# burchim/EfficientConformer

Measured on AMD Instinct MI355X. Metric: audio-frames/sec through encoder, EffConformerCTC-Small, 1/2/4/8 GPU, higher is better.
Workload: dtype bf16; 1 GPU; EfficientConformerCTCSmall: bf16 operands / fp32 accumulate, B=256 utterances/GPU (the largest single-GPU batch measured; SURVEY.md 8d lists B in {4, 32, 128}: --batch 128 is 0.79 x this rate, profiles/r5_31_bench_b128.json), lognormal 1.5-16 s (LibriSpeech-shaped), sorted desc; ragged: every utterance at its own length in one concatenated row space per row range (no pad frames; outputs = the refe; global_batch=256, streams_per_gpu=3, parallelism=dp1 (utterance shards), row_ranges=3 ragged row range(s) per GPU, cut for equal valid frames

## Files before the change

efficientconformer_amd/csrc/encoder.hip:

```cpp
#include "forward_common.h"
#include "pack.h"
#include "routes.h"

#include <cstring>

namespace {

thread_local std::string g_err;

}

int ec_fail(const char* msg) { g_err = msg ? msg : "error"; return -1; }

const void* ec_upload(EcEncoder* e, const void* src, size_t used) {
    if (e->dry) {
        static const char nowhere[16] = {0};
        const unsigned char* p = static_cast<const unsigned char*>(src);
        uint64_t h = 0xcbf29ce484222325ull ^ used;
        size_t i = 0;
        for (; i + 8 <= used; i += 8) { uint64_t w; memcpy(&w, p + i, 8); h = (h ^ w) * 0x100000001b3ull; h ^= h >> 29; }
        for (; i < used; ++i) h = (h ^ p[i]) * 0x100000001b3ull;
        e->dry->sum += h * 0x9E3779B97F4A7C15ull + 1; e->dry->buffers += 1; e->dry->bytes += (int64_t)used;
        return nowhere;
    }
// ... 12 lines not shown

int forward_dispatch(EcEncoder* e, const float* in, const int64_t* in_len, int from_audio, int n, const Shapes& s, float* out, int out_frames, int64_t* out_len,
                     void* workspace, size_t workspace_bytes, hipStream_t st) {
    char* ws = reinterpret_cast<char*>(workspace);
    const size_t mel_bytes = from_audio ? al((size_t)s.B * e->cfg.n_mels * s.Tm * 4) : 0;
    Workspace w; XWorkspace xw;
    size_t mel_off;
    if (e->exact_on) { xw = make_xworkspace(e, s); mel_off = xw.total; }
    else { w = make_workspace(e, s, from_audio != 0); mel_off = w.mel; }
    if (workspace_bytes < (e->exact_on ? xw.total + mel_bytes : w.total)) return fail("workspace too small");
    const float* mel = in;
    if (from_audio) {
        float* m = reinterpret_cast<float*>(ws + mel_off);
        PROF(PC_MEL, 0, (double)s.B * n * 4 + (double)s.B * e->cfg.n_mels * s.Tm * 4);
        EC_ABL(s.ragged && !e->exact_on ? 16 : 0, EC_TRY(launch_mel(in, s.B, n, e->mel, e->cfg.n_fft, e->cfg.hop_length, e->cfg.n_mels, s.Tm, e->cfg.normalize,
                                                                    e->cfg.mean, e->cfg.std, m, st, s.ragged ? in_len : nullptr)));
        mel = m;
    }
    if (e->exact_on) return forward_exact(e, mel, in_len, from_audio, s, xw, ws, out, out_len, st, out_frames);
    return forward_core(e, mel, in_len, from_audio, s, w, ws, out, out_len, st, out_frames);
}

bool ragged_host_lengths(const EcEncoder* e, const int64_t* host_len, int32_t batch, int32_t n, int32_t from_audio, std::vector<int>* tm) {
    tm->resize(batch);
    for (int b = 0; b < batch; ++b) {
        const int64_t l = host_len[b];
        if (l > n || (from_audio ? l <= e->cfg.n_fft / 2 : l < 1)) return false;
        (*tm)[b] = from_audio ? (int)(l / e->cfg.hop_length + 1) : (int)l;
    }
    return true;
}
// ... 110 lines not shown
    if (!x || !x_len || !x_len_host || !out || !workspace || batch <= 0 || n <= 0 || out_frames <= 0) return fail("bad argument");
    std::vector<int> tm;
    if (!ragged_host_lengths(e, x_len_host, batch, n, from_audio, &tm)) return fail("ragged lengths out of range (audio: n_fft / 2 < len <= n; mel: 1 <= len <= n)");
    Shapes s = make_shapes_ragged(e, tm);
    if (s.Tout.back() > out_frames) return fail("out_frames smaller than the longest utterance's output");
    s.Tm = from_audio ? n / e->cfg.hop_length + 1 : n;
    return forward_dispatch(e, x, x_len, from_audio, n, s, out, out_frames, out_len, workspace, workspace_bytes, (hipStream_t)stream);
}

int effconf_mel_frontend(EcEncoder* e, const float* audio, int32_t batch, int32_t n_samples, float* mel, void* stream) {
    if (!e || !e->finalized) return fail("encoder not finalized");
    if (!audio || !mel) return fail("mel_frontend: null argument");
    if (batch > 0 && n_samples <= e->cfg.n_fft / 2) return fail("mel_frontend: n_samples must exceed n_fft / 2 (reflect padding)");
    const int Tm = n_samples / e->cfg.hop_length + 1;
    EC_TRY(launch_mel(audio, batch, n_samples, e->mel, e->cfg.n_fft, e->cfg.hop_length, e->cfg.n_mels, Tm,
                      e->cfg.normalize, e->cfg.mean, e->cfg.std, mel, (hipStream_t)stream));
    return 0;
}

int effconf_ctc_greedy(EcEncoder* e, const float* enc_out, const int64_t* out_len, int32_t batch, int32_t t_out,
                       int32_t* labels, int32_t* label_len, float* logits, void* workspace, size_t workspace_bytes, void* stream) {
    if (!e || !e->finalized) return fail("encoder not finalized");
    if (!e->fc_wt) return fail("no CTC head (fc.weight / fc.bias) loaded");
    if (workspace_bytes < (size_t)batch * t_out * 4) return fail("workspace too small");
    int* preds = reinterpret_cast<int*>(workspace);
    hipStream_t st = (hipStream_t)stream;
    const int mode = e->exact_on && e->ctc_mfma == 2 ? 1 : e->ctc_mfma;
    if (mode == 2 && e->fc_hi && launch_ctc_split(enc_out, batch * t_out, e->blocks.back().dim_expand, e->fc_hi, e->fc_lo, e->fc_b, e->cfg.vocab_size,
                                                  preds, logits, st) == 0) {
    } else
    EC_TRY(launch_ctc_argmax(enc_out, batch * t_out, e->blocks.back().dim_expand, e->fc_wt, e->fc_b, e->cfg.vocab_size,
// ... 85 lines not shown
    e->ic_out.assign(probs, probs + n);
    return 0;
}

int effconf_encoder_set_option(EcEncoder* e, const char* name, int32_t value) {
    if (!e || !name) return fail("null argument");
    if (!strcmp(name, "fuse_subsample")) { if (value < 0 || value > 3) return fail("fuse_subsample: 0, 1, 2 or 3"); e->fuse_subsample = value; return 0; }
    if (!strcmp(name, "fuse_chain")) { e->fuse_chain = value != 0; return 0; }
    if (!strcmp(name, "ctc_mfma")) { if (value < 0 || value > 2) return fail("ctc_mfma: 0 (VALU), 1 (fp32 MFMA) or 2 (split-bf16 MFMA)"); e->ctc_mfma = value; return 0; }
    if (!strcmp(name, "wide_gemm")) { if (value < 0 || (value > 3 && value < 16)) return fail("wide_gemm: 0 (by shape), 1 (never), 2 (256-column tile), 3 (128-column tile), >= 16 (by shape with this many 256 x 256 tiles as the threshold)"); e->wide_gemm = value; return 0; }
    if (!strcmp(name, "attention_v2")) { if (value != 0 && value != 1 && value != 2) return fail("attention_v2: 0, 1 or 2"); e->attention_v2 = value; return 0; }
    if (!strcmp(name, "chain_full_max")) { if (value < 0 || value > 256) return fail("chain_full_max: widest stage (0..256) that runs chain A as ONE kernel"); e->chain_full_max = value; return 0; }
    if (!strcmp(name, "chain_max_dim")) { e->chain_max_dim = value; return 0; }
    if (!strcmp(name, "chain_small_m")) { e->chain_small_m = value; return 0; }
    if (!strcmp(name, "chain_pair")) { if (value != 0 && value != 5) return fail("chain_pair: 0 (chain.hip everywhere) or 5 (chain3.hip for chain A, chain2.hip for chain B at padded width 256)"); e->chain_pair = value; return 0; }
    if (!strcmp(name, "dwconv_mfma")) { if (value < 0 || value > 2) return fail("dwconv_mfma: 0, 1 (kernel size 15) or 2 (15 / 31 / 7)"); e->dwconv_mfma = value; return 0; }
    if (!strcmp(name, "tiled_min_k")) { e->tiled_min_k = value; return 0; }
    if (!strcmp(name, "tiled_auto")) { e->tiled_auto = value; return 0; }
    if (!strcmp(name, "split_ffn")) { e->split_ffn = value != 0; return 0; }
    if (!strcmp(name, "split_sublin")) { e->split_sublin = value != 0; return 0; }
    if (!strcmp(name, "sub3_auto")) { e->sub3_auto = value != 0; return 0; }
    if (!strcmp(name, "split_chain")) { e->split_chain = value != 0; return 0; }
    if (!strcmp(name, "trace_fused")) { e->trace_fused = value != 0; return 0; }
    if (!strcmp(name, "exact_attention")) { if (value < 0 || value > 2) return fail("exact_attention: 0 (tiled), 2 (tiled, 16-row workgroups) or 1 (one wave per query row)"); e->exact_attention = value; return 0; }
    if (!strcmp(name, "cache_pos_embeddings")) { e->e_cache_on = value != 0; e->e_cache.clear(); return 0; }
    if (!strcmp(name, "exact_fp32")) {
        if (!e->finalized) { e->exact_pack = e->exact_on = value != 0; e->exact_split = value == 2; return 0; }
        if (value && !e->exact_pack) return fail("exact_fp32 must be requested before effconf_encoder_finalize (the fp32 weights are uploaded there)");
        if (value == 2 && e->xsplit.empty()) return fail("exact_fp32 = 2 must be requested before effconf_encoder_finalize (the split weight images are built there)");
        e->exact_on = value != 0; e->exact_split = value == 2;
// ... 42 lines not shown
```

efficientconformer_amd/csrc/encoder_state.h:

```cpp
#pragma once
#include "kernels.h"
#include "../../include/effconf.h"

#include <map>
#include <string>
#include <vector>

int ec_fail(const char* msg);
inline int fail(const std::string& m) { return ec_fail(m.c_str()); }
#define EC_TRY(expr) do { int _rc = (expr); if (_rc != 0) return fail(std::string(#expr) + " failed rc=" + std::to_string(_rc)); } while (0)

inline int ld8(int d) { return ec_round_up(d, 8); }

struct HostTensor { std::vector<float> data; std::vector<int64_t> shape; };

struct PackedLinear { const bf16_t* w = nullptr; const float* bias = nullptr; int N = 0, K = 0, ldw = 0; std::vector<float> hbias;  };
struct SubChunkImg { const uint16_t *cimg = nullptr, *wimg = nullptr; const float* bias = nullptr; int ncb = 0, fo = 0; };
struct LNp { const float* g = nullptr; const float* b = nullptr; };

struct BlockW {
    LNp ln_ffn1, ln_att, ln_conv, ln_ffn2, ln_out;
    PackedLinear ffn1_a, ffn1_b, qkv, qkv_nat, pos, outp, pw1, pw2, res, ffn2_a, ffn2_b;
    const bf16_t *ffn1_bp = nullptr, *ffn2_bp = nullptr;
    const float *u = nullptr, *v = nullptr, *dw_w = nullptr, *dw_b = nullptr;
// ... 28 lines not shown
    PackDigest* dry = nullptr;
    size_t guard_bytes = 0;
    const float *sub_w9 = nullptr, *sub_b = nullptr;
    PackedLinear lin;
    const bf16_t* lin_fused = nullptr; int lin_fused_ld = 0;
    SubChunkImg sub3, xsub;
    const bf16_t* lin_rs = nullptr; const float* conv_tab = nullptr;
    int fuse_subsample = 2;
    bool fuse_chain = true;
    int ctc_mfma = 2;
    int attention_v2 = 1;
    int chain_full_max = 192;
    int dwconv_mfma = 1;
    int chain_pair = 5;
    int chain_small_m = 4096;
    int chain_max_dim = 256;
    int tiled_auto = 1;
    bool tiled_auto_on = false;
    int tiled_min_k = 256;
    std::vector<float*> att_out;
    int split_chain = 1;
    int sub3_auto = 1;
    int split_sublin = 1;
    int split_ffn = 1;
    bool trace_fused = false;
    int exact_attention = 0;
    const bf16_t* sub2_w = nullptr; const float* sub2_b = nullptr; int sub2_cp = 0;
    std::vector<BlockW> bw;
    const float *fc_wt = nullptr, *fc_b = nullptr;
    const bf16_t *fc_hi = nullptr, *fc_lo = nullptr;
// ... 51 lines not shown
```

efficientconformer_amd/csrc/forward_bf16.hip:

```cpp
#include "forward_common.h"
#include "routes.h"
#include "stream.h"

#include <cmath>

Workspace make_workspace(const EcEncoder* e, const Shapes& s, bool from_audio) {
    Workspace w;
    size_t off = 0;
    auto take = [&](size_t bytes) { size_t o = off; off += al(bytes); return o; };
    const size_t B = s.B;
    size_t mx = 0, ma = 0, mh = 0, mq = 0, me = 0, mg = 0, mc = 0;
    std::vector<size_t> esz;
    for (size_t k = 0; k < e->blocks.size(); ++k) {
        const EcBlock& b = e->blocks[k];
        const size_t T = s.Tin[k], D = b.dim_model, De = b.dim_expand;
        const size_t Tp = ec_round_up((int)T, b.group_size), Tg = Tp / b.group_size;
        const size_t d = (size_t)b.group_size * D / b.num_heads, dpad = ec_round_up((int)d, 32);
        const size_t Mi = (size_t)s.Min[k], Mo = (size_t)s.Mout[k], Mqk = (size_t)s.Mq[k];
        mx = std::max(mx, std::max(Mi * D, Mo * De) * 4);
        ma = std::max(ma, std::max(Mi * ld8(D), Mo * ld8(De)) * 2);
        mh = std::max(mh, std::max(Mi * D, Mo * De) * b.ff_ratio * 2);
        mq = std::max(mq, Mqk * D * 2 + 512);
        me = std::max(me, (size_t)b.num_heads * (2 * Tg - 1) * dpad * 2);
        esz.push_back((size_t)b.num_heads * (2 * Tg - 1) * dpad * 2 + 512);
// ... 92 lines not shown
    if (route == FRONT_TWO_LAYER) {
        const int T2 = (Tl1 - 1) / 2 + 1, F1 = c.n_mels / 2, F2q = c.n_mels / 4, C1 = c.sub_filters[1];
        { PROF(PC_SUBCONV, 2.0 * 9 * B * Tl1 * (double)C0 * F1, (double)B * c.n_mels * Tm * 4 + (double)B * Tl1 * F1 * e->sub2_cp * 2);
          EC_TRY(launch_subsample_conv_cl(mel, B, c.n_mels, Tm, Tl1, e->sub_w9, e->sub_b, C0, e->sub2_cp, act1, st, mel_len)); }
        trace_add(e, st, "subsample1", act1, (int64_t)B * F1 * Tl1, C0, e->sub2_cp, 1);
        { PROF(PC_GEMM_OTHER, 2.0 * 9 * (double)B * F2q * T2 * C0 * C1, (double)B * Tl1 * F1 * e->sub2_cp * 2 + (double)B * T2 * F2q * C1 * 2);
          EC_TRY(launch_conv2_igemm(act1, B, F1, Tl1, e->sub2_cp, e->sub2_w, 9 * e->sub2_cp, e->sub2_b, C1, F2q, T2, sub, st)); }
        trace_add(e, st, "subsample", sub, (int64_t)B * T2, F2q * C1, F2q * C1, 1);
        EC_TRY(run_gemm(e, PC_GEMM_OTHER, st, sub, F2q * C1, B * T2, e->lin, EPI_F32, rg ? xrect : x, N));
        if (rg) { PROF(PC_MISC, 0, Mr * N * 8); EC_TRY(launch_gather_rows(xrect, N, T2, r0, x, st)); }
    } else if (route == FRONT_CHUNKED) {
        PROF(PC_SUBCONV, 2.0 * 9 * Mr * Ksub + 2.0 * Mr * Ksub * N, (double)B * c.n_mels * Tm * 4 + Mr * N * 4);
        EC_TRY(launch_sublinear3(sub_chunk_params(e, e->sub3, mel, s, rg, x), st));
    } else if (route == FRONT_ROW_STAT) {
        PROF(PC_SUBCONV, 2.0 * 9 * Mr * Ksub + 2.0 * Mr * Ksub * N, (double)B * c.n_mels * Tm * 4 + Mr * N * 4);
        EC_ABL(rg ? 32 : 0, EC_TRY(launch_sublinear2(mel, B, c.n_mels, Tm, s.T1, e->conv_tab, e->lin_rs, e->lin.bias, C0, N, x, N, st, rg ? &r0 : nullptr, mel_len)));
    } else if (route == FRONT_TILED_FUSED) {
        PROF(PC_SUBCONV, 2.0 * 9 * Mr * Ksub + 2.0 * Mr * Ksub * N, (double)B * c.n_mels * Tm * 4 + Mr * N * 4);
        EC_TRY(launch_sublinear_fused(mel, B, c.n_mels, Tm, s.T1, e->sub_w9, e->sub_b, C0, e->lin_fused, e->lin_fused_ld, e->lin.bias, N, x, N, st));
    } else {
        const int Tcover = rg ? Tl1 + e->blocks[0].group_size - 1 : s.T1;
        { PROF(PC_SUBCONV, 2.0 * 9 * Mr * Ksub, (double)B * c.n_mels * Tm * 4 + Mr * Ksub * 2);
          EC_TRY(launch_subsample_conv(mel, B, c.n_mels, Tm, Tcover, e->sub_w9, e->sub_b, C0, sub, Ksub, st, mel_len, rg ? &r0 : nullptr)); }
        trace_add(e, st, "subsample", sub, s.Min[0], Ksub, Ksub, 1);
        EC_TRY(run_gemm(e, PC_GEMM_OTHER, st, sub, Ksub, (int)s.Min[0], e->lin, EPI_F32, x, N));
    }
    return 0;
}

ChainParams chain_params(const EcEncoder* e) { ChainParams cp{}; cp.small_m = e->chain_small_m; cp.pair = e->chain_pair; return cp; }

// ... 351 lines not shown
```

efficientconformer_amd/csrc/kernels.h:

```cpp
#pragma once
#include "common.h"

struct RaggedRows {
    const int* off;
    const int* len;
    int n;
    int rows;
    int tmax;
};

struct RaggedConv {
    const int *in_off, *in_len, *out_off, *out_len;
    const int* tile_off; int tiles;
    int n, out_rows;
};

enum GemmEpilogue {
    EPI_F32 = 0,
    EPI_BF16 = 1,
    EPI_SWISH_BF16 = 2,
    EPI_RESID_F32 = 3,
    EPI_GLU_BF16 = 4,
    EPI_QKV_NAT = 5,
};
// ... 97 lines not shown
int launch_relpos_attention(const AttnParams& p, hipStream_t s);
int launch_attention_probs(const AttnParams& p, float* att, hipStream_t s);
bool relpos_attention2_supported(int dpad);
int launch_relpos_attention2(const AttnParams& p, int waves, hipStream_t s);
int launch_attn_pad_rows_nat(const GemmParams& p, int B, hipStream_t s);
int launch_attn_pad_rows_ragged(bf16_t* qu, bf16_t* kh, bf16_t* vt, const float* u, int D, int G, const RaggedRows& rg, hipStream_t s);

int launch_subsample_conv(const float* mel, int B, int F, int Tm, int T1, const float* w9, const float* bias, int C,
                          bf16_t* out, int ldo, hipStream_t s, const int* rag_tm = nullptr, const RaggedRows* rg = nullptr);
int launch_gather_rows(const float* x, int D, int t_pitch, const RaggedRows& rg, float* out, hipStream_t s);
bool sublinear_fused_supported(int F, int N);
int launch_sublinear_fused(const float* mel, int B, int F, int Tm, int T1, const float* w9, const float* cbias, int C,
                           const bf16_t* W, int ldw, const float* bias, int N, float* out, int ldc, hipStream_t s);
int sublinear2_groups(int F, int C, int N);
int launch_sublinear2(const float* mel, int B, int F, int Tm, int T1, const float* ctab, const bf16_t* Wp, const float* bias, int C, int N,
                      float* out, int ldc, hipStream_t s, const RaggedRows* rg = nullptr, const int* rag_tm = nullptr);
int launch_subsample_conv_cl(const float* mel, int B, int F, int Tm, int T1, const float* w9, const float* bias, int C, int Cp,
                             bf16_t* out, hipStream_t s, const int* rag_tm = nullptr);
int launch_conv2_igemm(const bf16_t* act1, int B, int F1, int T1, int Cp, const bf16_t* W, int ldw, const float* bias,
                       int N, int F2, int T2, bf16_t* out, hipStream_t s);
int launch_dwconv(const bf16_t* g, int B, int T, int To, int C, int ld, const float* w_kc, const float* bias,
                  int ksize, int stride, bf16_t* out, hipStream_t s, const RaggedConv* rc = nullptr, int causal = 0,
                  const void* w_mfma = nullptr,
                  const void* w_mfma3 = nullptr);
int dwconv_mfma_groups(int ksize);
bool dwconv_mfma_supported(int ksize, int stride);
void pack_dwconv_mfma3(const float* w_kc, int ksize, int C, uint16_t* dst);
void pack_dwconv_mfma(const float* w_kc, int ksize, int C, uint16_t* dst);

struct ExGemmParams {
    const float* A; int lda;
// ... 100 lines not shown
int launch_sxf_dwconv(const float* g, int B, int T, int To, int C, const float* w_kc, const float* bias, int ks, int stride, float* out, hipStream_t s,
                      const RaggedConv* rc = nullptr, int causal = 0, int tcap_max = 0);
int launch_sxf_decimate(const float* x, int D, int stride, const RaggedConv& rc, float* out, hipStream_t s);
int launch_sxf_glu(const float* in, long long M, int N, float* out, hipStream_t s);

struct MelTables {
    const float* window;
    const float2* twiddle;
    const int* fb_start;
    const int* fb_count;
    const int* fb_offset;
    const float* fb_weight;
    int fb_nnz;
};
int launch_mel(const float* audio, int B, int L, const MelTables& t, int n_fft, int hop, int n_mels, int Tm,
               int normalize, float mean, float std, float* mel, hipStream_t s, const int64_t* ragged_len = nullptr);
int launch_mel_debug(int variant, int extra_lds, const float* audio, int B, int L, const MelTables& t, int n_fft, int hop, int n_mels,
                     int Tm, int normalize, float mean, float std, float* mel, unsigned int* dbg, hipStream_t s);
int launch_debug_neighbour(int kind, int blocks, int lds_bytes, int iters, float* buf, size_t n, hipStream_t s);
int launch_debug_spin(double microseconds, hipStream_t s);
int launch_debug_lds_fill(int mode, int blocks, int waves, const char* src, size_t window, int kib_per_wave, int passes, unsigned long long* out, hipStream_t s);
int launch_debug_victim(int kind, int blocks, int iters, float* out, hipStream_t s);
int launch_mel_debug_pk(int variant, int extra_lds, const float* audio, int B, int L, const MelTables& t, int n_fft, int hop, int n_mels,
                          int Tm, int normalize, float mean, float std, float* mel, unsigned int* dbg, hipStream_t s);

int launch_lengths(const int64_t* x_len, int B, int from_audio, int hop, int sub_layers, const int* block_stride,
                   int n_blocks, int* stage_lens , int64_t* out_len, hipStream_t s);
int launch_lengths_ragged(const int64_t* x_len, int B, int from_audio, int hop, int sub_layers, const int* block_stride, const int* group,
                          const int* heads, int n_blocks, int* stage_lens, int* mel_len, int* row_off, int* wg_off, int* tile_off,
                          int64_t* out_len, hipStream_t s);
int launch_ctc_argmax(const float* x, int M, int D, const float* Wt, const float* bias, int V,
// ... 7 lines not shown
```

efficientconformer_amd/csrc/mel.hip:

```cpp
#include "kernels.h"

#ifdef MEL_PK_BUILD
#define launch_mel launch_mel_pk_unused
#define launch_mel_debug launch_mel_debug_pk
#define MEL_NS mel_pk_build
#else
#define MEL_NS
#endif

namespace MEL_NS {

constexpr int NFFT = 512;
constexpr int FRAMES_PER_BLOCK = 32;
constexpr int MAX_MELS = 128;
constexpr int P1 = 72;
constexpr int P2 = 68;
constexpr int MAX_FBW = 768;

__device__ __forceinline__ float2 cmul(float2 a, float2 b) { return make_float2(a.x * b.x - a.y * b.y, a.x * b.y + a.y * b.x); }
__device__ __forceinline__ float2 cadd(float2 a, float2 b) { return make_float2(a.x + b.x, a.y + b.y); }
__device__ __forceinline__ float2 csub(float2 a, float2 b) { return make_float2(a.x - b.x, a.y - b.y); }
__device__ __forceinline__ float2 mul_mi(float2 a) { return make_float2(a.y, -a.x); }
__device__ __forceinline__ float2 mul_pi(float2 a) { return make_float2(-a.y, a.x); }

// ... 12 lines not shown
    {
        const float2 s0 = cadd(b[0], b[2]), s1 = cadd(b[1], b[3]), d0 = csub(b[0], b[2]), d1 = csub(b[1], b[3]);
        v[1] = cadd(s0, s1); v[5] = csub(s0, s1); v[3] = cadd(d0, mul_mi(d1)); v[7] = cadd(d0, mul_pi(d1));
    }
}

__device__ __forceinline__ float2 reread(const float2* p) {
    const volatile float* q = reinterpret_cast<const volatile float*>(p);
    return make_float2(q[0], q[1]);
}

template <int V, int MM>
__global__ __launch_bounds__(256) void mel_kernel(const float* __restrict__ audio, int L, MelTables tb, int hop,
                                                  int n_mels, int Tm, int normalize, float mean, float inv_std,
                                                  float* __restrict__ mel, unsigned int* __restrict__ dbg,
                                                  const int64_t* __restrict__ rag_len = nullptr) {
    constexpr int CAN = (V & 1) ? 512 : 0;
    constexpr int WBUF = 8 * P1 * 8;
    constexpr int O_SBUF = CAN * 4, O_POST = O_SBUF + 4 * WBUF, O_STW = O_POST + CAN * 4, O_SWIN = O_STW + (NFFT / 2) * 8,
                  O_SOUT = O_SWIN + NFFT * 4, O_SFW = O_SOUT + MM * (FRAMES_PER_BLOCK + 1) * 4, O_END = O_SFW + MAX_FBW * 4;
    static_assert(8 * P1 >= NFFT && P1 >= P2 && 8 * P1 * 2 >= 264 + NFFT / 2 + 1, "one buffer holds Z[512], the step-2 layout and the two power spectra");
    __shared__ __attribute__((aligned(16))) char lds[O_END];
    float2* stw = reinterpret_cast<float2*>(lds + O_STW);
    float* swin = reinterpret_cast<float*>(lds + O_SWIN);
    float (*sout)[FRAMES_PER_BLOCK + 1] = reinterpret_cast<float (*)[FRAMES_PER_BLOCK + 1]>(lds + O_SOUT);
    float* sfw = reinterpret_cast<float*>(lds + O_SFW);
    if constexpr ((V & 1) != 0) {
        unsigned int* c0 = reinterpret_cast<unsigned int*>(lds), *c1 = reinterpret_cast<unsigned int*>(lds + O_POST);
        for (int i = threadIdx.x; i < CAN; i += 256) { c0[i] = 0xC0FFEE00u + i; c1[i] = 0xBADC0DE0u + i; }
    }
    auto hand_off = [&]() __attribute__((always_inline)) { if constexpr ((V & 4) != 0) __syncthreads(); else wave_sync(); };
// ... 8 lines not shown
    const bool fw_lds = tb.fb_nnz <= MAX_FBW;
    {
        static_assert(NFFT == 512 && MAX_FBW == 768, "two / three passes of 256 threads");
        const float2 w = tb.twiddle[tid];
        const float wn0 = tb.window[tid], wn1 = tb.window[tid + 256];
        float f[3];
#pragma unroll
        for (int j = 0; j < 3; ++j) { const int i = tid + 256 * j; f[j] = tb.fb_weight[i < tb.fb_nnz ? i : (tb.fb_nnz > 0 ? tb.fb_nnz - 1 : 0)]; }
        stw[tid] = w;
        swin[tid] = wn0; swin[tid + 256] = wn1;
        if (fw_lds) {
#pragma unroll
            for (int j = 0; j < 3; ++j) if (tid + 256 * j < tb.fb_nnz) sfw[tid + 256 * j] = f[j];
        }
    }
    int fs0[2], fcnt[2], foff[2];
#pragma unroll
    for (int j = 0; j < 2; ++j) {
        const int m = (threadIdx.x & 63) + 64 * j, mc = m < n_mels ? m : n_mels - 1;
        fs0[j] = tb.fb_start[mc]; fcnt[j] = m < n_mels ? tb.fb_count[mc] : 0; foff[j] = tb.fb_offset[mc];
    }
    __syncthreads();
    float2* A = reinterpret_cast<float2*>(lds + O_SBUF + wave * WBUF);
    float2* B = A;
    auto tw = [&](int m) __attribute__((always_inline)) {
        float2 w = stw[m & 255];
        const uint32_t sg = (uint32_t)(m & 256) << 23;
        w.x = __uint_as_float(__float_as_uint(w.x) ^ sg); w.y = __uint_as_float(__float_as_uint(w.y) ^ sg);
        return w;
    };
    const float* a = audio + (size_t)b * L;

    auto gather = [&](int ta, float (&xa)[8], float (&xb)[8]) __attribute__((always_inline)) {
#pragma unroll
        for (int j = 0; j < 8; ++j) {
            const int n = lane + 64 * j;
            int sa = ta * hop - NFFT / 2 + n, sb = sa + hop;
            sa = sa < 0 ? -sa : sa; sa = sa >= Lb ? 2 * (Lb - 1) - sa : sa; sa = sa < 0 ? 0 : (sa >= Lb ? Lb - 1 : sa);
            sb = sb < 0 ? -sb : sb; sb = sb >= Lb ? 2 * (Lb - 1) - sb : sb; sb = sb < 0 ? 0 : (sb >= Lb ? Lb - 1 : sb);
            xa[j] = a[sa]; xb[j] = a[sb];
        }
    };
    float nxa[8], nxb[8];
    gather(t0 + wave * (FRAMES_PER_BLOCK / 4), nxa, nxb);
    for (int it = 0; it < FRAMES_PER_BLOCK / 8; ++it) {
        const int fl = wave * (FRAMES_PER_BLOCK / 4) + 2 * it;
        const int ta = t0 + fl, tbb = ta + 1;
        float2 v[8];
#pragma unroll
        for (int j = 0; j < 8; ++j) {
            const float w = swin[lane + 64 * j];
            v[j] = make_float2(ta < Tmb ? nxa[j] * w : 0.f, tbb < Tmb ? nxb[j] * w : 0.f);
        }
        bool nza = false, nzb = false;
#pragma unroll
        for (int j = 0; j < 8; ++j) { nza |= v[j].x != 0.f; nzb |= v[j].y != 0.f; }
        const bool live_a = __builtin_amdgcn_ballot_w64(nza) != 0, live_b = __builtin_amdgcn_ballot_w64(nzb) != 0;
        if (it + 1 < FRAMES_PER_BLOCK / 8) gather(ta + 2, nxa, nxb);
        {
            const int n2 = lane >> 3;
            dft8(v);
#pragma unroll
            for (int k1 = 0; k1 < 8; ++k1) { v[k1] = cmul(v[k1], tw((8 * n2 * k1) & 511)); A[k1 * P1 + lane] = v[k1]; }
        }
        hand_off();
        if constexpr ((V & 2) != 0) {
#pragma unroll
            for (int k1 = 0; k1 < 8; ++k1) bad[1] += neq(A[k1 * P1 + lane], v[k1]);
        }
        {
            const int k1 = lane >> 3, n3 = lane & 7;
#pragma unroll
            for (int n2 = 0; n2 < 8; ++n2) v[n2] = A[k1 * P1 + n2 * 8 + n3];
// ... 42 lines not shown
        hand_off();
#pragma unroll
        for (int j = 0; j < 5; ++j) {
            const int k = lane + 64 * j;
            if (k <= NFFT / 2) {
                const float2 z = zz[j], zc = zcc[j];
                const float ar = 0.5f * (z.x + zc.x), ai = 0.5f * (z.y - zc.y);
                const float br = 0.5f * (z.y + zc.y), bi = 0.5f * (zc.x - z.x);
                Pa[k] = live_a ? ar * ar + ai * ai : 0.f;
                Pb[k] = live_b ? br * br + bi * bi : 0.f;
            }
        }
        hand_off();
#pragma unroll
        for (int mj = 0; mj < 2; ++mj) {
            const int m = lane + 64 * mj;
            if (m >= n_mels) break;
            const int s0 = fs0[mj], cnt = fcnt[mj], off = foff[mj];
            float ya = 0.f, yb = 0.f;
            if (fw_lds) {
                for (int j0 = 0; j0 < cnt; j0 += 4) {
                    float wj[4], pa[4], pb[4];
#pragma unroll
                    for (int e = 0; e < 4; ++e) {
                        const int j = j0 + e, jc = j < cnt ? j : cnt - 1;
                        wj[e] = j < cnt ? sfw[off + jc] : 0.f;
                        pa[e] = Pa[s0 + jc]; pb[e] = Pb[s0 + jc];
                    }
#pragma unroll
                    for (int e = 0; e < 4; ++e) { ya = fmaf(pa[e], wj[e], ya); yb = fmaf(pb[e], wj[e], yb); }
                }
            } else {
// ... 16 lines not shown
        const unsigned int* c0 = reinterpret_cast<const unsigned int*>(lds), *c1 = reinterpret_cast<const unsigned int*>(lds + O_POST);
        for (int i = threadIdx.x; i < CAN; i += 256) bad[0] += (c0[i] != 0xC0FFEE00u + i) + (c1[i] != 0xBADC0DE0u + i);
    }
    if constexpr (V != 0) {
#pragma unroll
        for (int i = 0; i < 8; ++i) if (bad[i]) atomicAdd(dbg + i, bad[i]);
    }
}

}
#ifdef MEL_PK_BUILD
using namespace mel_pk_build;
#endif

int launch_mel(const float* audio, int B, int L, const MelTables& t, int n_fft, int hop, int n_mels, int Tm,
               int normalize, float mean, float std, float* mel, hipStream_t s, const int64_t* ragged_len) {
    if (B <= 0) return 0;
    if (n_fft != NFFT || n_mels > MAX_MELS || L <= n_fft / 2) return -2;
    const int tiles = (Tm + FRAMES_PER_BLOCK - 1) / FRAMES_PER_BLOCK;
    if (n_mels <= 80)
        hipLaunchKernelGGL((mel_kernel<0, 80>), dim3(B * tiles), dim3(256), 0, s, audio, L, t, hop, n_mels, Tm, normalize, mean,
                           1.0f / std, mel, (unsigned int*)nullptr, ragged_len);
    else
        hipLaunchKernelGGL((mel_kernel<0, MAX_MELS>), dim3(B * tiles), dim3(256), 0, s, audio, L, t, hop, n_mels, Tm, normalize, mean,
                           1.0f / std, mel, (unsigned int*)nullptr, ragged_len);
    return hipGetLastError() == hipSuccess ? 0 : -1;
}

#if defined(EFFCONF_DEBUG_ABI) || defined(MEL_PK_BUILD)
int launch_mel_debug(int variant, int extra_lds, const float* audio, int B, int L, const MelTables& t, int n_fft, int hop, int n_mels,
                     int Tm, int normalize, float mean, float std, float* mel, unsigned int* dbg, hipStream_t s) {
    if (B <= 0) return 0;
    if (n_fft != NFFT || n_mels > MAX_MELS || L <= n_fft / 2) return -2;
#ifndef MEL_PK_BUILD
    if (variant & 8) return launch_mel_debug_pk(variant & 7, extra_lds, audio, B, L, t, n_fft, hop, n_mels, Tm, normalize, mean, std, mel, dbg, s);
#endif
    const int tiles = (Tm + FRAMES_PER_BLOCK - 1) / FRAMES_PER_BLOCK;
#define MEL_DBG_CASE(VV) case VV: { static LdsAttr attr; ensure_dynamic_lds(reinterpret_cast<const void*>(&mel_kernel<VV, MAX_MELS>), extra_lds, attr); \
        hipLaunchKernelGGL((mel_kernel<VV, MAX_MELS>), dim3(B * tiles), dim3(256), extra_lds, s, audio, L, t, hop, n_mels, Tm, normalize, mean, 1.0f / std, mel, dbg, (const int64_t*)nullptr); break; }
    switch (variant) {
        MEL_DBG_CASE(0) MEL_DBG_CASE(1) MEL_DBG_CASE(2) MEL_DBG_CASE(3) MEL_DBG_CASE(4) MEL_DBG_CASE(5) MEL_DBG_CASE(6) MEL_DBG_CASE(7)
        default: return -2;
    }
#undef MEL_DBG_CASE
    return hipGetLastError() == hipSuccess ? 0 : -1;
}
#endif
```

efficientconformer_amd/csrc/sublinear2.hip:

```cpp
#include "kernels.h"
#include "rowstat.h"

namespace {

template <int NT>
__device__ __forceinline__ void store_rows(char* yb, size_t pitch, int N, int m_base, int M, char* stg, int lane, const f32x16 (&xc)[NT]) {
    const int lr = lane & 31, half = lane >> 5;
#pragma unroll
    for (int w = 0; w < (NT + 1) / 2; ++w) {
        wave_sync();
#pragma unroll
        for (int tt = 0; tt < 2; ++tt) {
            const int t = 2 * w + tt;
            if (t < NT) {
#pragma unroll
                for (int q = 0; q < 4; ++q)
                    *reinterpret_cast<float4*>(stg + lr * STG_ROW + (tt * 32 + q * 8 + half * 4) * 4) =
                        make_float4(xc[t][4 * q + 0], xc[t][4 * q + 1], xc[t][4 * q + 2], xc[t][4 * q + 3]);
            }
        }
        wave_sync();
        stage_store(stg, yb, pitch, N * 4, m_base, M, 256 * w, lane);
    }
}

__device__ __forceinline__ void glds4(const void* g, char* lds_wave_base) {
    const uint32_t l = (uint32_t)(uintptr_t)(lds_void_t*)lds_wave_base;
    asm volatile("s_mov_b32 m0, %0\n\ts_nop 0\n\tglobal_load_lds_dword %1, off" ::"s"(l), "v"(g) : "memory", "m0");
}

__device__ __forceinline__ uint32_t split_hi(float x) { return __float_as_uint(x) & 0xFFFF0000u; }

template <int CG, int NT, int NBUF, int NW>
__global__ __launch_bounds__(NW * 64, NW == 8 ? 2 : 1) void sublinear2_kernel(const float* __restrict__ mel, int F, int Tm, int T1, int M,
                                                            const float* __restrict__ ctab , const bf16_t* __restrict__ Wp,
                                                            const float* __restrict__ bias, int N, float* __restrict__ out, int ldc,
                                                            const int* __restrict__ rag_off, const int* __restrict__ rag_t1, const int* __restrict__ rag_tm, int rag_n) {
    constexpr int KSF = 2 * CG, P1 = 2 * KSF;
    constexpr int SLAB = NT * CH * P1 * 16;
    constexpr int NDMA = NT * CH * P1 / 64, PER = NDMA / NW;
    static_assert(NDMA % NW == 0, "uniform DMA count per wave");
    extern __shared__ __attribute__((aligned(16))) char smem[];
    const int tid = threadIdx.x, lane = tid & 63;
    const int wave = __builtin_amdgcn_readfirstlane(tid >> 6);
    const int lr = lane & 31, half = lane >> 5;
    const int m_base = (blockIdx.x * NW + wave) * 32;
    const int F2 = F / 2;
    const int ldw = P1 * 8;

    uint32_t doff[PER];
#pragma unroll
    for (int k = 0; k < PER; ++k) {
        const int i = wave + NW * k;
        const int sub = i / (P1 / 2), ii = i - sub * (P1 / 2);
        doff[k] = (uint32_t)(sub * CH * ldw) * 2u + dma_rows32_off<P1>(ldw, ii, lane);
    }
// ... 29 lines not shown
    if (rag_off) {
        b = ragged_find(rag_off, rag_n, mc); t = mc - rag_off[b]; tmb = rag_tm[b];
        pad_row = t >= rag_t1[b];
        t = pad_row ? 0 : t;
    } else { b = mc / T1; t = mc - b * T1; }
    const float* melb = mel + (size_t)b * F * Tm;
    int col[3]; bool cok[3];
#pragma unroll
    for (int j = 0; j < 3; ++j) { const int tc = 2 * t - 1 + j; cok[j] = tc >= 0 && tc < tmb; col[j] = tc < 0 ? 0 : (tc < tmb ? tc : tmb - 1); }
    auto row_ptr = [&](int fr) { return melb + (size_t)(fr < 0 ? 0 : (fr < F ? fr : F - 1)) * Tm; };
    auto mask_row = [&](int fr, float (&r)[3]) __attribute__((always_inline)) {
        const bool ok = fr >= 0 && fr < F;
#pragma unroll
        for (int j = 0; j < 3; ++j) r[j] = (ok && cok[j]) ? r[j] : 0.f;
    };
    char* mstage = smem + NBUF * SLAB + wave * (2 * 6 * 256);
    auto issue_rows = [&](int fr, int slot) __attribute__((always_inline)) {
        const float* p0 = row_ptr(fr);
        const float* p1 = row_ptr(fr + 1);
#pragma unroll
        for (int j = 0; j < 3; ++j) glds4(p0 + col[j], mstage + (slot * 6 + j) * 256);
#pragma unroll
        for (int j = 0; j < 3; ++j) glds4(p1 + col[j], mstage + (slot * 6 + 3 + j) * 256);
    };
    float r0[3], r1[3], r2[3];
    {
        const float* pa = row_ptr(-1); const float* pb = row_ptr(0); const float* pc = row_ptr(1);
#pragma unroll
        for (int j = 0; j < 3; ++j) { r0[j] = pa[col[j]]; r1[j] = pb[col[j]]; r2[j] = pc[col[j]]; }
#pragma unroll
        for (int j = 0; j < 3; ++j) asm volatile("" :: "v"(r0[j]), "v"(r1[j]), "v"(r2[j]));
        mask_row(-1, r0); mask_row(0, r1); mask_row(1, r2);
    }
    issue_rows(2, 0);
#pragma unroll
    for (int c = 0; c < NBUF - 1; ++c)
        if (c < F2) issue(c);

    f32x16 xc[NT];
#pragma unroll
    for (int nt = 0; nt < NT; ++nt)
#pragma unroll
        for (int r = 0; r < 16; ++r) xc[nt][r] = 0.f;

    const int q0 = (half + lr) % P1;
    for (int f = 0; f < F2; ++f) {
        if (NBUF >= 3 && f + 1 < F2) wait_vmcnt<PER>(); else wait_vmcnt<0>();
        wg_barrier();
        float n1[3], n2[3];
        {
            const float* st = reinterpret_cast<const float*>(mstage + (f & 1) * 6 * 256) + lane;
#pragma unroll
            for (int j = 0; j < 3; ++j) { n1[j] = st[j * 64]; n2[j] = st[(3 + j) * 64]; }
        }
        mask_row(2 * f + 2, n1); mask_row(2 * f + 3, n2);
        float tp[8];
        if (half == 0) { tp[0] = r0[0]; tp[1] = r0[1]; tp[2] = r0[2]; tp[3] = r1[0]; tp[4] = r1[1]; tp[5] = r1[2]; tp[6] = r2[0]; tp[7] = r2[1]; }
        else { tp[0] = r2[2]; tp[1] = 1.0f; tp[2] = 0.f; tp[3] = 0.f; tp[4] = 0.f; tp[5] = 0.f; tp[6] = 0.f; tp[7] = 0.f; }
        uint32_t ph[4], pl[4];
#pragma unroll
        for (int e = 0; e < 4; ++e) {
            const uint32_t h0 = split_hi(tp[2 * e]), h1 = split_hi(tp[2 * e + 1]);
            ph[e] = (h0 >> 16) | h1;
            pl[e] = pack_bf2(tp[2 * e] - __uint_as_float(h0), tp[2 * e + 1] - __uint_as_float(h1));
        }
        const bf16x8 phi = as_bf16x8(make_uint4(ph[0], ph[1], ph[2], ph[3])), plo = as_bf16x8(make_uint4(pl[0], pl[1], pl[2], pl[3]));
#pragma unroll
        for (int j = 0; j < 3; ++j) { r0[j] = r2[j]; r1[j] = n1[j]; r2[j] = n2[j]; }
// ... 2 lines not shown
        if (f + NBUF - 1 < F2) issue(f + NBUF - 1);

        bf16x8 xf[KSF];
#pragma unroll
        for (int g = 0; g < CG; ++g) {
            f32x16 cv;
#pragma unroll
            for (int r = 0; r < 16; ++r) cv[r] = 0.f;
            cv = __builtin_amdgcn_mfma_f32_32x32x16_bf16(whi[g], phi, cv, 0, 0, 0);
            cv = __builtin_amdgcn_mfma_f32_32x32x16_bf16(whi[g], plo, cv, 0, 0, 0);
            cv = __builtin_amdgcn_mfma_f32_32x32x16_bf16(wlo[g], phi, cv, 0, 0, 0);
#pragma unroll
            for (int j = 0; j < 2; ++j) {
                float y[8];
#pragma unroll
                for (int e = 0; e < 8; ++e) y[e] = swishf_(cv[8 * j + e]);
                xf[2 * g + j] = as_bf16x8(make_uint4(pack_bf2(y[0], y[1]), pack_bf2(y[2], y[3]), pack_bf2(y[4], y[5]), pack_bf2(y[6], y[7])));
            }
        }
        const char* buf = smem + (f % NBUF) * SLAB + lr * (P1 * 16);
#pragma unroll
        for (int nt = 0; nt < NT; ++nt) {
            const char* w = buf + nt * CH * P1 * 16;
            constexpr int FB = 4;
#pragma unroll
            for (int s0 = 0; s0 < KSF; s0 += FB) {
                bf16x8 wa[FB];
#pragma unroll
                for (int i = 0; i < FB; ++i) {
                    int q = q0 + 2 * (s0 + i);
                    q -= q >= P1 ? P1 : 0;
// ... 6 lines not shown
    }
    wait_vmcnt<0>();
    __syncthreads();
#pragma unroll
    for (int nt = 0; nt < NT; ++nt)
#pragma unroll
        for (int q = 0; q < 4; ++q) {
            const int n = nt * 32 + q * 8 + half * 4;
            const float4 bz = *reinterpret_cast<const float4*>(bias + n);
            xc[nt][4 * q + 0] += bz.x; xc[nt][4 * q + 1] += bz.y; xc[nt][4 * q + 2] += bz.z; xc[nt][4 * q + 3] += bz.w;
            if (pad_row) { xc[nt][4 * q + 0] = 0.f; xc[nt][4 * q + 1] = 0.f; xc[nt][4 * q + 2] = 0.f; xc[nt][4 * q + 3] = 0.f; }
        }
    store_rows<NT>(reinterpret_cast<char*>(out), (size_t)ldc * 4, N, m_base, M, smem + wave * STG_BYTES, lane, xc);
}

template <int CG, int NT, int NBUF, int NW>
int launch2(const float* mel, int B, int F, int Tm, int T1, const float* ctab, const bf16_t* Wp, const float* bias, int N, float* out, int ldc,
            hipStream_t s, const RaggedRows* rg, const int* rag_tm) {
    constexpr int P1 = 4 * CG, SLAB = NT * CH * P1 * 16;
    const int M = rg ? rg->rows : B * T1;
    const int lds = NBUF * SLAB + NW * 2 * 6 * 256 > NW * STG_BYTES ? NBUF * SLAB + NW * 2 * 6 * 256 : NW * STG_BYTES;
    if (lds > 160 * 1024) return -4;
    static LdsAttr attr;
    ensure_dynamic_lds(reinterpret_cast<const void*>(&sublinear2_kernel<CG, NT, NBUF, NW>), lds, attr);
    hipLaunchKernelGGL((sublinear2_kernel<CG, NT, NBUF, NW>), dim3((M + NW * 32 - 1) / (NW * 32)), dim3(NW * 64), lds, s, mel, F, Tm, T1, M, ctab, Wp, bias, N, out, ldc,
                       rg ? rg->off : nullptr, rg ? rg->len : nullptr, rag_tm, rg ? rg->n : 0);
    return hipGetLastError() == hipSuccess ? 0 : -1;
}

}

int sublinear2_groups(int F, int C, int N) {
    if (F != 80 || N % 4) return 0;
    if (C <= 128 && N <= 128) return 4;
    if (C <= 192 && N <= 192) return 6;
    return 0;
}

int launch_sublinear2(const float* mel, int B, int F, int Tm, int T1, const float* ctab, const bf16_t* Wp, const float* bias, int C, int N,
                      float* out, int ldc, hipStream_t s, const RaggedRows* rg, const int* rag_tm) {
    if (B <= 0 || T1 <= 0) return 0;
    if (rg && (!rag_tm || rg->rows <= 0)) return rg->rows <= 0 ? 0 : -2;
    switch (sublinear2_groups(F, C, N)) {
        case 4: return launch2<4, 4, 3, 8>(mel, B, F, Tm, T1, ctab, Wp, bias, N, out, ldc, s, rg, rag_tm);
        case 6: return launch2<6, 6, 2, 4>(mel, B, F, Tm, T1, ctab, Wp, bias, N, out, ldc, s, rg, rag_tm);
    }
    return -2;
}
```

Before: 61.23 million mel-frames/s (valid, 10 ms hop).

## Add fast front-end paths for mel STFT gathering and sublinear2 row staging

Adds a front_fast option, on by default, that changes two front-end kernels. In the mel kernel, interior frames gather audio with direct strided loads and skip the per-element bounds masks, and the two mel passes are swapped when there are more than 64 mels. In sublinear2, each half-wave now stages only one mel row per slot, which halves the staging LDS and the DMA issue count. It also templates on the number of live quads in the last channel group, so swish is not computed for padded channels. This cuts redundant loads and ALU work in the front end, at the cost of more template instantiations and extra code paths whose correctness depends on the ragged boundaries being handled right.

```diff
diff --git a/efficientconformer_amd/csrc/encoder.hip b/efficientconformer_amd/csrc/encoder.hip
--- a/efficientconformer_amd/csrc/encoder.hip
+++ b/efficientconformer_amd/csrc/encoder.hip
@@ -50,7 +50,7 @@
         float* m = reinterpret_cast<float*>(ws + mel_off);
         PROF(PC_MEL, 0, (double)s.B * n * 4 + (double)s.B * e->cfg.n_mels * s.Tm * 4);
         EC_ABL(s.ragged && !e->exact_on ? 16 : 0, EC_TRY(launch_mel(in, s.B, n, e->mel, e->cfg.n_fft, e->cfg.hop_length, e->cfg.n_mels, s.Tm, e->cfg.normalize,
-                                                                    e->cfg.mean, e->cfg.std, m, st, s.ragged ? in_len : nullptr)));
+                                                                    e->cfg.mean, e->cfg.std, m, st, s.ragged ? in_len : nullptr, e->front_fast)));
         mel = m;
     }
     if (e->exact_on) return forward_exact(e, mel, in_len, from_audio, s, xw, ws, out, out_len, st, out_frames);
@@ -191,7 +191,7 @@
     if (batch > 0 && n_samples <= e->cfg.n_fft / 2) return fail("mel_frontend: n_samples must exceed n_fft / 2 (reflect padding)");
     const int Tm = n_samples / e->cfg.hop_length + 1;
     EC_TRY(launch_mel(audio, batch, n_samples, e->mel, e->cfg.n_fft, e->cfg.hop_length, e->cfg.n_mels, Tm,
-                      e->cfg.normalize, e->cfg.mean, e->cfg.std, mel, (hipStream_t)stream));
+                      e->cfg.normalize, e->cfg.mean, e->cfg.std, mel, (hipStream_t)stream, nullptr, e->front_fast));
     return 0;
 }
 
@@ -307,6 +307,7 @@
     if (!strcmp(name, "chain_max_dim")) { e->chain_max_dim = value; return 0; }
     if (!strcmp(name, "chain_small_m")) { e->chain_small_m = value; return 0; }
     if (!strcmp(name, "chain_pair")) { if (value != 0 && value != 5) return fail("chain_pair: 0 (chain.hip everywhere) or 5 (chain3.hip for chain A, chain2.hip for chain B at padded width 256)"); e->chain_pair = value; return 0; }
+    if (!strcmp(name, "front_fast")) { e->front_fast = value != 0; return 0; }
     if (!strcmp(name, "dwconv_mfma")) { if (value < 0 || value > 2) return fail("dwconv_mfma: 0, 1 (kernel size 15) or 2 (15 / 31 / 7)"); e->dwconv_mfma = value; return 0; }
     if (!strcmp(name, "tiled_min_k")) { e->tiled_min_k = value; return 0; }
     if (!strcmp(name, "tiled_auto")) { e->tiled_auto = value; return 0; }
diff --git a/efficientconformer_amd/csrc/encoder_state.h b/efficientconformer_amd/csrc/encoder_state.h
--- a/efficientconformer_amd/csrc/encoder_state.h
+++ b/efficientconformer_amd/csrc/encoder_state.h
@@ -66,6 +66,7 @@
     int dwconv_mfma = 1;
     int chain_pair = 5;
     int chain_small_m = 4096;
+    int front_fast = 1;
     int chain_max_dim = 256;
     int tiled_auto = 1;
     bool tiled_auto_on = false;
diff --git a/efficientconformer_amd/csrc/forward_bf16.hip b/efficientconformer_amd/csrc/forward_bf16.hip
--- a/efficientconformer_amd/csrc/forward_bf16.hip
+++ b/efficientconformer_amd/csrc/forward_bf16.hip
@@ -130,7 +130,7 @@
         EC_TRY(launch_sublinear3(sub_chunk_params(e, e->sub3, mel, s, rg, x), st));
     } else if (route == FRONT_ROW_STAT) {
         PROF(PC_SUBCONV, 2.0 * 9 * Mr * Ksub + 2.0 * Mr * Ksub * N, (double)B * c.n_mels * Tm * 4 + Mr * N * 4);
-        EC_ABL(rg ? 32 : 0, EC_TRY(launch_sublinear2(mel, B, c.n_mels, Tm, s.T1, e->conv_tab, e->lin_rs, e->lin.bias, C0, N, x, N, st, rg ? &r0 : nullptr, mel_len)));
+        EC_ABL(rg ? 32 : 0, EC_TRY(launch_sublinear2(mel, B, c.n_mels, Tm, s.T1, e->conv_tab, e->lin_rs, e->lin.bias, C0, N, x, N, st, rg ? &r0 : nullptr, mel_len, e->front_fast)));
     } else if (route == FRONT_TILED_FUSED) {
         PROF(PC_SUBCONV, 2.0 * 9 * Mr * Ksub + 2.0 * Mr * Ksub * N, (double)B * c.n_mels * Tm * 4 + Mr * N * 4);
         EC_TRY(launch_sublinear_fused(mel, B, c.n_mels, Tm, s.T1, e->sub_w9, e->sub_b, C0, e->lin_fused, e->lin_fused_ld, e->lin.bias, N, x, N, st));
diff --git a/efficientconformer_amd/csrc/kernels.h b/efficientconformer_amd/csrc/kernels.h
--- a/efficientconformer_amd/csrc/kernels.h
+++ b/efficientconformer_amd/csrc/kernels.h
@@ -135,7 +135,7 @@
                            const bf16_t* W, int ldw, const float* bias, int N, float* out, int ldc, hipStream_t s);
 int sublinear2_groups(int F, int C, int N);
 int launch_sublinear2(const float* mel, int B, int F, int Tm, int T1, const float* ctab, const bf16_t* Wp, const float* bias, int C, int N,
-                      float* out, int ldc, hipStream_t s, const RaggedRows* rg = nullptr, const int* rag_tm = nullptr);
+                      float* out, int ldc, hipStream_t s, const RaggedRows* rg = nullptr, const int* rag_tm = nullptr, int fast = 1);
 int launch_subsample_conv_cl(const float* mel, int B, int F, int Tm, int T1, const float* w9, const float* bias, int C, int Cp,
                              bf16_t* out, hipStream_t s, const int* rag_tm = nullptr);
 int launch_conv2_igemm(const bf16_t* act1, int B, int F1, int T1, int Cp, const bf16_t* W, int ldw, const float* bias,
@@ -266,7 +266,7 @@
     int fb_nnz;
 };
 int launch_mel(const float* audio, int B, int L, const MelTables& t, int n_fft, int hop, int n_mels, int Tm,
-               int normalize, float mean, float std, float* mel, hipStream_t s, const int64_t* ragged_len = nullptr);
+               int normalize, float mean, float std, float* mel, hipStream_t s, const int64_t* ragged_len = nullptr, int fast = 1);
 int launch_mel_debug(int variant, int extra_lds, const float* audio, int B, int L, const MelTables& t, int n_fft, int hop, int n_mels,
                      int Tm, int normalize, float mean, float std, float* mel, unsigned int* dbg, hipStream_t s);
 int launch_debug_neighbour(int kind, int blocks, int lds_bytes, int iters, float* buf, size_t n, hipStream_t s);
diff --git a/efficientconformer_amd/csrc/mel.hip b/efficientconformer_amd/csrc/mel.hip
--- a/efficientconformer_amd/csrc/mel.hip
+++ b/efficientconformer_amd/csrc/mel.hip
@@ -50,7 +50,7 @@
 __global__ __launch_bounds__(256) void mel_kernel(const float* __restrict__ audio, int L, MelTables tb, int hop,
                                                   int n_mels, int Tm, int normalize, float mean, float inv_std,
                                                   float* __restrict__ mel, unsigned int* __restrict__ dbg,
-                                                  const int64_t* __restrict__ rag_len = nullptr) {
+                                                  const int64_t* __restrict__ rag_len = nullptr, int fast = 0) {
     constexpr int CAN = (V & 1) ? 512 : 0;
     constexpr int WBUF = 8 * P1 * 8;
     constexpr int O_SBUF = CAN * 4, O_POST = O_SBUF + 4 * WBUF, O_STW = O_POST + CAN * 4, O_SWIN = O_STW + (NFFT / 2) * 8,
@@ -89,11 +89,14 @@
             for (int j = 0; j < 3; ++j) if (tid + 256 * j < tb.fb_nnz) sfw[tid + 256 * j] = f[j];
         }
     }
+    const bool swap_passes = fast && n_mels > 64;
+    const int mbase[2] = {swap_passes ? n_mels - 64 : 0, swap_passes ? 0 : 64};
+    const int mlim[2] = {n_mels, swap_passes ? n_mels - 64 : n_mels};
     int fs0[2], fcnt[2], foff[2];
 #pragma unroll
     for (int j = 0; j < 2; ++j) {
-        const int m = (threadIdx.x & 63) + 64 * j, mc = m < n_mels ? m : n_mels - 1;
-        fs0[j] = tb.fb_start[mc]; fcnt[j] = m < n_mels ? tb.fb_count[mc] : 0; foff[j] = tb.fb_offset[mc];
+        const int m = (threadIdx.x & 63) + mbase[j], mc = m < mlim[j] ? m : mlim[j] - 1;
+        fs0[j] = tb.fb_start[mc]; fcnt[j] = m < mlim[j] ? tb.fb_count[mc] : 0; foff[j] = tb.fb_offset[mc];
     }
     __syncthreads();
     float2* A = reinterpret_cast<float2*>(lds + O_SBUF + wave * WBUF);
@@ -116,22 +119,40 @@
             xa[j] = a[sa]; xb[j] = a[sb];
         }
     };
+    const int wave_u = __builtin_amdgcn_readfirstlane(wave);
+    auto interior = [&](int ta) __attribute__((always_inline)) { return V == 0 && fast && ta * hop >= NFFT / 2 && (ta + 1) * hop + NFFT / 2 <= Lb; };
+    auto gather_pair = [&](int ta, float (&xa)[8], float (&xb)[8]) __attribute__((always_inline)) {
+        if (interior(ta)) {
+            const float* pa = a + (ta * hop - NFFT / 2) + lane;
+            const float* pb = pa + hop;
+#pragma unroll
+            for (int j = 0; j < 8; ++j) { xa[j] = pa[64 * j]; xb[j] = pb[64 * j]; }
+        } else gather(ta, xa, xb);
+    };
     float nxa[8], nxb[8];
-    gather(t0 + wave * (FRAMES_PER_BLOCK / 4), nxa, nxb);
+    gather_pair(t0 + wave_u * (FRAMES_PER_BLOCK / 4), nxa, nxb);
     for (int it = 0; it < FRAMES_PER_BLOCK / 8; ++it) {
-        const int fl = wave * (FRAMES_PER_BLOCK / 4) + 2 * it;
+        const int fl = wave_u * (FRAMES_PER_BLOCK / 4) + 2 * it;
         const int ta = t0 + fl, tbb = ta + 1;
         float2 v[8];
-#pragma unroll
-        for (int j = 0; j < 8; ++j) {
-            const float w = swin[lane + 64 * j];
-            v[j] = make_float2(ta < Tmb ? nxa[j] * w : 0.f, tbb < Tmb ? nxb[j] * w : 0.f);
+        if (interior(ta)) {
+#pragma unroll
+            for (int j = 0; j < 8; ++j) {
+                const float w = swin[lane + 64 * j];
+                v[j] = make_float2(nxa[j] * w, nxb[j] * w);
+            }
+        } else {
+#pragma unroll
+            for (int j = 0; j < 8; ++j) {
+                const float w = swin[lane + 64 * j];
+                v[j] = make_float2(ta < Tmb ? nxa[j] * w : 0.f, tbb < Tmb ? nxb[j] * w : 0.f);
+            }
         }
         bool nza = false, nzb = false;
 #pragma unroll
         for (int j = 0; j < 8; ++j) { nza |= v[j].x != 0.f; nzb |= v[j].y != 0.f; }
         const bool live_a = __builtin_amdgcn_ballot_w64(nza) != 0, live_b = __builtin_amdgcn_ballot_w64(nzb) != 0;
-        if (it + 1 < FRAMES_PER_BLOCK / 8) gather(ta + 2, nxa, nxb);
+        if (it + 1 < FRAMES_PER_BLOCK / 8) gather_pair(ta + 2, nxa, nxb);
         {
             const int n2 = lane >> 3;
             dft8(v);
@@ -204,8 +225,8 @@
         hand_off();
 #pragma unroll
         for (int mj = 0; mj < 2; ++mj) {
-            const int m = lane + 64 * mj;
-            if (m >= n_mels) break;
+            const int m = lane + mbase[mj];
+            if (m >= mlim[mj]) break;
             const int s0 = fs0[mj], cnt = fcnt[mj], off = foff[mj];
             float ya = 0.f, yb = 0.f;
             if (fw_lds) {
@@ -252,16 +273,16 @@
 #endif
 
 int launch_mel(const float* audio, int B, int L, const MelTables& t, int n_fft, int hop, int n_mels, int Tm,
-               int normalize, float mean, float std, float* mel, hipStream_t s, const int64_t* ragged_len) {
+               int normalize, float mean, float std, float* mel, hipStream_t s, const int64_t* ragged_len, int fast) {
     if (B <= 0) return 0;
     if (n_fft != NFFT || n_mels > MAX_MELS || L <= n_fft / 2) return -2;
     const int tiles = (Tm + FRAMES_PER_BLOCK - 1) / FRAMES_PER_BLOCK;
     if (n_mels <= 80)
         hipLaunchKernelGGL((mel_kernel<0, 80>), dim3(B * tiles), dim3(256), 0, s, audio, L, t, hop, n_mels, Tm, normalize, mean,
-                           1.0f / std, mel, (unsigned int*)nullptr, ragged_len);
+                           1.0f / std, mel, (unsigned int*)nullptr, ragged_len, fast);
     else
         hipLaunchKernelGGL((mel_kernel<0, MAX_MELS>), dim3(B * tiles), dim3(256), 0, s, audio, L, t, hop, n_mels, Tm, normalize, mean,
-                           1.0f / std, mel, (unsigned int*)nullptr, ragged_len);
+                           1.0f / std, mel, (unsigned int*)nullptr, ragged_len, fast);
     return hipGetLastError() == hipSuccess ? 0 : -1;
 }
 
@@ -275,7 +296,7 @@
 #endif
     const int tiles = (Tm + FRAMES_PER_BLOCK - 1) / FRAMES_PER_BLOCK;
 #define MEL_DBG_CASE(VV) case VV: { static LdsAttr attr; ensure_dynamic_lds(reinterpret_cast<const void*>(&mel_kernel<VV, MAX_MELS>), extra_lds, attr); \
-        hipLaunchKernelGGL((mel_kernel<VV, MAX_MELS>), dim3(B * tiles), dim3(256), extra_lds, s, audio, L, t, hop, n_mels, Tm, normalize, mean, 1.0f / std, mel, dbg, (const int64_t*)nullptr); break; }
+        hipLaunchKernelGGL((mel_kernel<VV, MAX_MELS>), dim3(B * tiles), dim3(256), extra_lds, s, audio, L, t, hop, n_mels, Tm, normalize, mean, 1.0f / std, mel, dbg, (const int64_t*)nullptr, 0); break; }
     switch (variant) {
         MEL_DBG_CASE(0) MEL_DBG_CASE(1) MEL_DBG_CASE(2) MEL_DBG_CASE(3) MEL_DBG_CASE(4) MEL_DBG_CASE(5) MEL_DBG_CASE(6) MEL_DBG_CASE(7)
         default: return -2;
diff --git a/efficientconformer_amd/csrc/sublinear2.hip b/efficientconformer_amd/csrc/sublinear2.hip
--- a/efficientconformer_amd/csrc/sublinear2.hip
+++ b/efficientconformer_amd/csrc/sublinear2.hip
@@ -31,7 +31,7 @@
 
 __device__ __forceinline__ uint32_t split_hi(float x) { return __float_as_uint(x) & 0xFFFF0000u; }
 
-template <int CG, int NT, int NBUF, int NW>
+template <int CG, int NT, int NBUF, int NW, int LQ, int RP>
 __global__ __launch_bounds__(NW * 64, NW == 8 ? 2 : 1) void sublinear2_kernel(const float* __restrict__ mel, int F, int Tm, int T1, int M,
                                                             const float* __restrict__ ctab , const bf16_t* __restrict__ Wp,
                                                             const float* __restrict__ bias, int N, float* __restrict__ out, int ldc,
@@ -40,6 +40,7 @@
     constexpr int SLAB = NT * CH * P1 * 16;
     constexpr int NDMA = NT * CH * P1 / 64, PER = NDMA / NW;
     static_assert(NDMA % NW == 0, "uniform DMA count per wave");
+    static_assert((RP == 3 || RP == 6) && LQ >= 0 && LQ <= 4, "row pieces per frequency; live quads of the last group");
     extern __shared__ __attribute__((aligned(16))) char smem[];
     const int tid = threadIdx.x, lane = tid & 63;
     const int wave = __builtin_amdgcn_readfirstlane(tid >> 6);
@@ -99,14 +100,20 @@
 #pragma unroll
         for (int j = 0; j < 3; ++j) r[j] = (ok && cok[j]) ? r[j] : 0.f;
     };
-    char* mstage = smem + NBUF * SLAB + wave * (2 * 6 * 256);
+    char* mstage = smem + NBUF * SLAB + wave * (2 * RP * 256);
     auto issue_rows = [&](int fr, int slot) __attribute__((always_inline)) {
         const float* p0 = row_ptr(fr);
         const float* p1 = row_ptr(fr + 1);
-#pragma unroll
-        for (int j = 0; j < 3; ++j) glds4(p0 + col[j], mstage + (slot * 6 + j) * 256);
-#pragma unroll
-        for (int j = 0; j < 3; ++j) glds4(p1 + col[j], mstage + (slot * 6 + 3 + j) * 256);
+        if constexpr (RP == 3) {
+            const float* ph = half ? p1 : p0;
+#pragma unroll
+            for (int j = 0; j < 3; ++j) glds4(ph + col[j], mstage + (slot * 3 + j) * 256);
+        } else {
+#pragma unroll
+            for (int j = 0; j < 3; ++j) glds4(p0 + col[j], mstage + (slot * 6 + j) * 256);
+#pragma unroll
+            for (int j = 0; j < 3; ++j) glds4(p1 + col[j], mstage + (slot * 6 + 3 + j) * 256);
+        }
     };
     float r0[3], r1[3], r2[3];
     {
@@ -134,9 +141,15 @@
         wg_barrier();
         float n1[3], n2[3];
         {
-            const float* st = reinterpret_cast<const float*>(mstage + (f & 1) * 6 * 256) + lane;
-#pragma unroll
-            for (int j = 0; j < 3; ++j) { n1[j] = st[j * 64]; n2[j] = st[(3 + j) * 64]; }
+            if constexpr (RP == 3) {
+                const float* st = reinterpret_cast<const float*>(mstage + (f & 1) * 3 * 256) + lr;
+#pragma unroll
+                for (int j = 0; j < 3; ++j) { n1[j] = st[j * 64]; n2[j] = st[j * 64 + 32]; }
+            } else {
+                const float* st = reinterpret_cast<const float*>(mstage + (f & 1) * 6 * 256) + lane;
+#pragma unroll
+                for (int j = 0; j < 3; ++j) { n1[j] = st[j * 64]; n2[j] = st[(3 + j) * 64]; }
+            }
         }
         mask_row(2 * f + 2, n1); mask_row(2 * f + 3, n2);
         float tp[8];
@@ -169,7 +182,7 @@
             for (int j = 0; j < 2; ++j) {
                 float y[8];
 #pragma unroll
-                for (int e = 0; e < 8; ++e) y[e] = swishf_(cv[8 * j + e]);
+                for (int e = 0; e < 8; ++e) y[e] = (g == CG - 1 && 2 * j + e / 4 >= LQ) ? 0.f : swishf_(cv[8 * j + e]);
                 xf[2 * g + j] = as_bf16x8(make_uint4(pack_bf2(y[0], y[1]), pack_bf2(y[2], y[3]), pack_bf2(y[4], y[5]), pack_bf2(y[6], y[7])));
             }
         }
@@ -206,16 +219,16 @@
     store_rows<NT>(reinterpret_cast<char*>(out), (size_t)ldc * 4, N, m_base, M, smem + wave * STG_BYTES, lane, xc);
 }
 
-template <int CG, int NT, int NBUF, int NW>
+template <int CG, int NT, int NBUF, int NW, int LQ, int RP>
 int launch2(const float* mel, int B, int F, int Tm, int T1, const float* ctab, const bf16_t* Wp, const float* bias, int N, float* out, int ldc,
             hipStream_t s, const RaggedRows* rg, const int* rag_tm) {
     constexpr int P1 = 4 * CG, SLAB = NT * CH * P1 * 16;
     const int M = rg ? rg->rows : B * T1;
-    const int lds = NBUF * SLAB + NW * 2 * 6 * 256 > NW * STG_BYTES ? NBUF * SLAB + NW * 2 * 6 * 256 : NW * STG_BYTES;
+    const int lds = NBUF * SLAB + NW * 2 * RP * 256 > NW * STG_BYTES ? NBUF * SLAB + NW * 2 * RP * 256 : NW * STG_BYTES;
     if (lds > 160 * 1024) return -4;
     static LdsAttr attr;
-    ensure_dynamic_lds(reinterpret_cast<const void*>(&sublinear2_kernel<CG, NT, NBUF, NW>), lds, attr);
-    hipLaunchKernelGGL((sublinear2_kernel<CG, NT, NBUF, NW>), dim3((M + NW * 32 - 1) / (NW * 32)), dim3(NW * 64), lds, s, mel, F, Tm, T1, M, ctab, Wp, bias, N, out, ldc,
+    ensure_dynamic_lds(reinterpret_cast<const void*>(&sublinear2_kernel<CG, NT, NBUF, NW, LQ, RP>), lds, attr);
+    hipLaunchKernelGGL((sublinear2_kernel<CG, NT, NBUF, NW, LQ, RP>), dim3((M + NW * 32 - 1) / (NW * 32)), dim3(NW * 64), lds, s, mel, F, Tm, T1, M, ctab, Wp, bias, N, out, ldc,
                        rg ? rg->off : nullptr, rg ? rg->len : nullptr, rag_tm, rg ? rg->n : 0);
     return hipGetLastError() == hipSuccess ? 0 : -1;
 }
@@ -230,12 +243,21 @@
 }
 
 int launch_sublinear2(const float* mel, int B, int F, int Tm, int T1, const float* ctab, const bf16_t* Wp, const float* bias, int C, int N,
-                      float* out, int ldc, hipStream_t s, const RaggedRows* rg, const int* rag_tm) {
+                      float* out, int ldc, hipStream_t s, const RaggedRows* rg, const int* rag_tm, int fast) {
     if (B <= 0 || T1 <= 0) return 0;
     if (rg && (!rag_tm || rg->rows <= 0)) return rg->rows <= 0 ? 0 : -2;
-    switch (sublinear2_groups(F, C, N)) {
-        case 4: return launch2<4, 4, 3, 8>(mel, B, F, Tm, T1, ctab, Wp, bias, N, out, ldc, s, rg, rag_tm);
-        case 6: return launch2<6, 6, 2, 4>(mel, B, F, Tm, T1, ctab, Wp, bias, N, out, ldc, s, rg, rag_tm);
-    }
+    const int groups = sublinear2_groups(F, C, N);
+    const int live = C - 32 * (groups - 1), lq = live <= 0 ? 0 : (live >= 32 ? 4 : (live + 7) / 8);
+#define EC_SUB2(CG, NT, NBUF, NW, LQ, RP) return launch2<CG, NT, NBUF, NW, LQ, RP>(mel, B, F, Tm, T1, ctab, Wp, bias, N, out, ldc, s, rg, rag_tm)
+#define EC_SUB2_LQ(CG, NT, NBUF, NW) \
+    if (!fast) EC_SUB2(CG, NT, NBUF, NW, 4, 6); \
+    switch (lq) { case 0: EC_SUB2(CG, NT, NBUF, NW, 0, 3); case 1: EC_SUB2(CG, NT, NBUF, NW, 1, 3); case 2: EC_SUB2(CG, NT, NBUF, NW, 2, 3); \
+                  case 3: EC_SUB2(CG, NT, NBUF, NW, 3, 3); default: EC_SUB2(CG, NT, NBUF, NW, 4, 3); }
+    switch (groups) {
+        case 4: EC_SUB2_LQ(4, 4, 3, 8)
+        case 6: EC_SUB2_LQ(6, 6, 2, 4)
+    }
+#undef EC_SUB2_LQ
+#undef EC_SUB2
     return -2;
 }
```

Result: no change. 61.81 million mel-frames/s (valid, 10 ms hop) (median of 6 runs) (+0.9%).
